# rlvc/FEALESS

Hardware: AMD Instinct MI355X
Metric: frames/sec (640x480 RGB-D x N templates, 20 ICP iters) (higher is better)
Workload: dtype u8

## Files before the change

fealess_amd/csrc/fl_frontend.hip:

```cpp
#include "fl_internal.h"
#include <float.h>

#ifndef FL_CQ_DOT4
#define FL_CQ_DOT4 1
#endif

__device__ __forceinline__ int clampi(int v, int lo, int hi) { return v < lo ? lo : (v > hi ? hi : v); }
__device__ __forceinline__ int reflect101(int p, int len)
{
  if (len == 1) return 0;
  while (p < 0 || p >= len) p = p < 0 ? -p : 2 * len - 2 - p;
  return p;
}

__device__ __forceinline__ float fast_atan2_deg(float y, float x)
{
  const float p1 = 0.9997878412794807f * (float)(180 / 3.14159265358979323846);
  const float p3 = -0.3258083974640975f * (float)(180 / 3.14159265358979323846);
  const float p5 = 0.1555786518463281f * (float)(180 / 3.14159265358979323846);
  const float p7 = -0.04432655554792128f * (float)(180 / 3.14159265358979323846);
  const float ax = fabsf(x), ay = fabsf(y);
  const bool steep = !(ax >= ay);
  const float c = (steep ? ax : ay) / ((steep ? ay : ax) + (float)DBL_EPSILON);
  const float c2 = c * c;
  const float poly = (((p7 * c2 + p5) * c2 + p3) * c2 + p1) * c;
  float a = steep ? 90.f - poly : poly;
  if (x < 0) a = 180.f - a;
  if (y < 0) a = 360.f - a;
  return a;
}

#define CQ_COLS 60
#define CQ_CH 60

__device__ __forceinline__ unsigned wave_from_prev(unsigned v) { return (unsigned)__builtin_amdgcn_update_dpp((int)v, (int)v, 0x138, 0xF, 0xF, false); }
__device__ __forceinline__ unsigned wave_from_next(unsigned v) { return (unsigned)__builtin_amdgcn_update_dpp((int)v, (int)v, 0x130, 0xF, 0xF, false); }
__device__ __forceinline__ unsigned wave_from_prev0(unsigned v) { return (unsigned)__builtin_amdgcn_update_dpp(0, (int)v, 0x138, 0xF, 0xF, true); }
__device__ __forceinline__ unsigned wave_from_next0(unsigned v) { return (unsigned)__builtin_amdgcn_update_dpp(0, (int)v, 0x130, 0xF, 0xF, true); }

__host__ __device__ __forceinline__ void cq_window_addr(uint32_t row_mis, int w, int xc, uint32_t *off, uint32_t *shift, int *first)
{
  const int f = xc - 3 < 0 ? 0 : (xc - 3 > w - 7 ? w - 7 : xc - 3);
  const uint32_t o = row_mis + 3u * (uint32_t)f;
  *off = o & ~3u;
  *shift = o & 3u;
  *first = f;
}

__host__ __device__ __forceinline__ uint32_t cq_alignbyte(uint32_t hi, uint32_t lo, uint32_t s)
{
#if defined(__HIP_DEVICE_COMPILE__)
  return __builtin_amdgcn_alignbyte(hi, lo, s);
#else
  return (uint32_t)((((uint64_t)hi << 32) | lo) >> (8 * (s & 3u)));
#endif
}

__host__ __device__ __forceinline__ void cq_window(const uint8_t *__restrict__ row4, uint32_t row_mis, int w, int xc, bool any_left,
                                                   bool any_right, uint32_t *wd)
{
  uint32_t off, shift;
  int first;
  cq_window_addr(row_mis, w, xc, &off, &shift, &first);
  const int dpx = xc - 3 - first;
  uint32_t d[6];
  const uint8_t *q = (const uint8_t *)__builtin_assume_aligned(row4 + off, 4);
  __builtin_memcpy(d, q, 16);
  __builtin_memcpy(d + 4, q + 16, 8);
#pragma unroll
  for (int k = 0; k < 5; ++k) wd[k] = cq_alignbyte(d[k + 1], d[k], shift);
  wd[5] = cq_alignbyte(d[5], d[5], shift);
#define CQ_TAKE(e0, e1, e2, e3, e4, e5, e6, e7, e8)                                                                                 \
  {                                                                                                                                 \
    const bool b0 = (dw & 1u) != 0u, b1 = (dw & 2u) != 0u;                                                                          \
    const uint32_t t0 = b0 ? e1 : e0, t1 = b0 ? e2 : e1, t2 = b0 ? e3 : e2, t3 = b0 ? e4 : e3, t4 = b0 ? e5 : e4, t5 = b0 ? e6 : e5, \
                   t6 = b0 ? e7 : e6, t7 = b0 ? e8 : e7;                                                                            \
    const uint32_t g0 = b1 ? t2 : t0, g1 = b1 ? t3 : t1, g2 = b1 ? t4 : t2, g3 = b1 ? t5 : t3, g4 = b1 ? t6 : t4, g5 = b1 ? t7 : t5; \
    wd[0] = cq_alignbyte(g1, g0, s);                                                                                                \
    wd[1] = cq_alignbyte(g2, g1, s);                                                                                                \
    wd[2] = cq_alignbyte(g3, g2, s);                                                                                                \
    wd[3] = cq_alignbyte(g4, g3, s);                                                                                                \
    wd[4] = cq_alignbyte(g5, g4, s);                                                                                                \
    wd[5] = cq_alignbyte(g5, g5, s);                                                                                                \
  }
  if (any_left) {
    const uint32_t s = dpx < 0 ? (uint32_t)-dpx : 0u, dw = 3u - s;
    const uint32_t p = wd[0] & 0xFFFFFFu;
    CQ_TAKE((p | (p << 24)), ((p >> 8) | (p << 16)), ((p >> 16) | (p << 8)), wd[0], wd[1], wd[2], wd[3], wd[4], wd[5])
  }
  if (any_right) {
    const uint32_t n = dpx > 0 ? 3u * (uint32_t)dpx : 0u, dw = n >> 2, s = n & 3u;
    const uint32_t p = (wd[4] >> 16) | ((wd[5] & 0xFFu) << 16);
    CQ_TAKE(wd[0], wd[1], wd[2], wd[3], wd[4], ((p >> 16) | (p << 8)), (p | (p << 24)), ((p >> 8) | (p << 16)), 0u)
  }
#undef CQ_TAKE
}

template <bool kNarrow>
__device__ __forceinline__ void cq_hrow(const uint8_t *__restrict__ src, int w, int h, int row, int xc, bool any_left, bool any_right,
                                        int *h3)
{
  const int kk[7] = {8, 28, 56, 72, 56, 28, 8};
  const uint8_t *p = src + (size_t)clampi(row, 0, h - 1) * (size_t)(w * 3);
  int a0 = 0, a1 = 0, a2 = 0;
  if (!kNarrow) {
    const uint32_t mis = (uint32_t)(uintptr_t)p & 3u;
    uint32_t wd[6];
    cq_window(p - mis, mis, w, xc, any_left, any_right, wd);
#if FL_CQ_DOT4
    unsigned acc[3] = {0u, 0u, 0u};
#pragma unroll
    for (int ch = 0; ch < 3; ++ch)
#pragma unroll
      for (int k = 0; k < 6; ++k) {
        unsigned wk = 0;
#pragma unroll
        for (int t = 0; t < 7; ++t)
          if (((3 * t + ch) >> 2) == k) wk |= (unsigned)kk[t] << (8 * ((3 * t + ch) & 3));
        if (wk != 0u) acc[ch] = __builtin_amdgcn_udot4(wd[k], wk, acc[ch], false);
      }
    a0 = (int)acc[0]; a1 = (int)acc[1]; a2 = (int)acc[2];
#else
#pragma unroll
    for (int t = 0; t < 7; ++t) {
      const int b0 = 3 * t, b1 = 3 * t + 1, b2 = 3 * t + 2;
      a0 += kk[t] * (int)((wd[b0 >> 2] >> (8 * (b0 & 3))) & 0xFFu);
      a1 += kk[t] * (int)((wd[b1 >> 2] >> (8 * (b1 & 3))) & 0xFFu);
      a2 += kk[t] * (int)((wd[b2 >> 2] >> (8 * (b2 & 3))) & 0xFFu);
    }
#endif
  } else {
#pragma unroll
    for (int t = 0; t < 7; ++t) {
      const uint8_t *q = p + 3 * clampi(xc + t - 3, 0, w - 1);
      a0 += kk[t] * q[0];
      a1 += kk[t] * q[1];
      a2 += kk[t] * q[2];
    }
  }
  h3[0] = a0;
  h3[1] = a1;
  h3[2] = a2;
}

extern "C" void fl_dev_cq_window_addr(unsigned row_mis, int w, int xc, unsigned *off, unsigned *shift, int *first)
{
  cq_window_addr(row_mis, w, xc, off, shift, first);
}
extern "C" void fl_dev_cq_window_taps(const uint8_t *row4, unsigned row_mis, int w, int xc, int any_left, int any_right, uint8_t *taps21)
{
  uint32_t wd[6];
  cq_window(row4, row_mis, w, xc, any_left != 0, any_right != 0, wd);
  for (int b = 0; b < 21; ++b) taps21[b] = (uint8_t)(wd[b >> 2] >> (8 * (b & 3)));
}

#ifndef FL_CQ_WPE
#define FL_CQ_WPE 6
#endif
template <bool kMag, bool kNarrow>
__global__ __launch_bounds__(256) __attribute__((amdgpu_waves_per_eu(kNarrow ? 6 : FL_CQ_WPE, kNarrow ? 6 : FL_CQ_WPE))) void k_color_quantize(const uint8_t *__restrict__ bgr, size_t in_stride,
                                                        uint8_t *__restrict__ dst, size_t out_stride, int w, int h,
                                                        float threshold_sq, int nstrips, int nchunks, int chunk_rows,
                                                        float *__restrict__ mag_out, const uint32_t *__restrict__ tiles,
                                                        size_t tiles_stride)
{
  const int wave = __builtin_amdgcn_readfirstlane((int)(threadIdx.x >> 6)), lane = threadIdx.x & 63;
  const int item = blockIdx.x * 4 + wave;
  if (item >= nstrips * nchunks) return;
  const int strip = item % nstrips, chunk = item / nstrips;
  int row_lo = 0, row_hi = h - 1;
  if (tiles) {
    const uint32_t *tb = tiles + (size_t)blockIdx.z * tiles_stride;
    const int t = chunk * nstrips + strip;
    if (!((tb[FL_TILE_WORDS + (t >> 5)] >> (t & 31)) & 1u)) return;
    const uint32_t rw = tb[2 * FL_TILE_WORDS + 32 * FL_TILE_WORDS + t];
    row_lo = (int)(rw >> 16);
    row_hi = (int)(rw & 0xFFFFu);
  }
  const uint8_t *src = bgr + (size_t)blockIdx.z * in_stride;
  uint8_t *out = dst + (size_t)blockIdx.z * out_stride;
  const int x = strip * CQ_COLS + lane - 2;
  const int xc = clampi(x, 0, w - 1);
  const int y0 = max(chunk * chunk_rows, row_lo), y1 = min(min(h, chunk * chunk_rows + chunk_rows), row_hi + 1);
  if (y0 >= y1) return;
  const bool any_left = strip == 0, any_right = strip * CQ_COLS + 61 > w - 4;

  int H[7][3];
  {
    const int center = clampi(y0 - 2, 0, h - 1);
#pragma unroll
    for (int i = 0; i < 7; ++i) cq_hrow<kNarrow>(src, w, h, center + i - 3, xc, any_left, any_right, H[i]);
  }
  uint32_t Sl[3] = {0, 0, 0}, Sc[3] = {0, 0, 0}, Sr[3] = {0, 0, 0};
  uint32_t Qp[3] = {0, 0, 0};
  float Mg[3] = {0.f, 0.f, 0.f};
  auto smooth = [&](int p) __attribute__((always_inline)) {
    uint32_t vv[3];
#pragma unroll
    for (int ch = 0; ch < 3; ++ch)
      vv[ch] = __umul24(8u, (unsigned)(H[p % 7][ch] + H[(p + 6) % 7][ch])) + __umul24(28u, (unsigned)(H[(p + 1) % 7][ch] + H[(p + 5) % 7][ch])) +
               __umul24(56u, (unsigned)(H[(p + 2) % 7][ch] + H[(p + 4) % 7][ch])) + __umul24(72u, (unsigned)H[(p + 3) % 7][ch]);
    const uint32_t S = (uint32_t)(((int)vv[0] + (1 << 15)) >> 16) | ((uint32_t)(((int)vv[1] + (1 << 15)) >> 16) << 8) |
                       ((uint32_t)(((int)vv[2] + (1 << 15)) >> 16) << 16);
    const uint32_t L = wave_from_prev0(S), R = wave_from_next0(S);
    Sl[0] = Sl[1]; Sl[1] = Sl[2]; Sl[2] = L;
    Sc[0] = Sc[1]; Sc[1] = Sc[2]; Sc[2] = S;
    Sr[0] = Sr[1]; Sr[1] = Sr[2]; Sr[2] = R;
  };
  auto again = [&]() __attribute__((always_inline)) {
    Sl[0] = Sl[1]; Sl[1] = Sl[2];
    Sc[0] = Sc[1]; Sc[1] = Sc[2];
    Sr[0] = Sr[1]; Sr[1] = Sr[2];
  };
  auto finish = [&](int yv) __attribute__((always_inline)) {
    if (yv < y0) return;
    const int ys = yv - 1;
    int bdx = 0, bdy = 0, bmag = 0;
    {
      int dxs[3], dys[3], mags[3];
#pragma unroll
      for (int ch = 0; ch < 3; ++ch) {
        const int sh = 8 * ch;
#define PX(v) ((int)(((v) >> sh) & 0xFFu))
        const int dx = (PX(Sr[0]) - PX(Sl[0])) + 2 * (PX(Sr[1]) - PX(Sl[1])) + (PX(Sr[2]) - PX(Sl[2]));
        const int dy = (PX(Sl[2]) - PX(Sl[0])) + 2 * (PX(Sc[2]) - PX(Sc[0])) + (PX(Sr[2]) - PX(Sr[0]));
#undef PX
        dxs[ch] = dx;
        dys[ch] = dy;
        mags[ch] = __mul24(dx, dx) + __mul24(dy, dy);
      }
      if (mags[0] >= mags[1] && mags[0] >= mags[2]) { bdx = dxs[0]; bdy = dys[0]; bmag = mags[0]; }
      else if (mags[1] >= mags[0] && mags[1] >= mags[2]) { bdx = dxs[1]; bdy = dys[1]; bmag = mags[1]; }
      else { bdx = dxs[2]; bdy = dys[2]; bmag = mags[2]; }
    }
    const float ang = fast_atan2_deg((float)bdy, (float)bdx);
    int qi = __float2int_rn(ang * (float)(16.0 / 360.0));
    qi = qi < 0 ? 0 : (qi > 255 ? 255 : qi);
    const bool inside = ys > 0 && ys < h - 1 && x > 0 && x < w - 1;
    const uint32_t q = inside ? (uint32_t)(qi & 7) : 0u;
    const uint32_t oh = 1u << (4 * q);
    const uint32_t ohl = wave_from_prev0(oh), ohr = wave_from_next0(oh);
    Qp[0] = Qp[1]; Qp[1] = Qp[2]; Qp[2] = oh + ohl + ohr;
    Mg[0] = Mg[1]; Mg[1] = Mg[2]; Mg[2] = (float)bmag;
    if (yv < y0 + 2) return;
    const int yo = yv - 2;
    if (lane >= 2 && lane < 2 + CQ_COLS && x < w && yo < y1) {
      uint8_t res = 0;
      if (yo >= 1 && yo < h - 1 && x >= 1 && x < w - 1 && Mg[1] > threshold_sq) {
        const unsigned hist = Qp[0] + Qp[1] + Qp[2];
        const unsigned maj = (hist + 0x33333333u) & 0x88888888u;
        if (maj) res = (uint8_t)(1u << ((__ffs((int)maj) - 4) >> 2));
      }
      out[(size_t)yo * w + x] = res;
      if (kMag) mag_out[(size_t)blockIdx.z * out_stride + (size_t)yo * w + x] = Mg[1];
      else if (mag_out) mag_out[(size_t)yo * w + x] = Mg[1];
    }
  };

  const int ylast = y1 + 1, yadv = min(ylast, h - 1);
  int yv = y0 - 2;
  smooth(0);
  for (++yv; yv <= min(ylast, 0); ++yv) {
    again();
    finish(yv);
  }
  for (;;) {
#pragma unroll
    for (int P = 0; P < 7; ++P) {
      if (yv > yadv) goto below;
      cq_hrow<kNarrow>(src, w, h, yv + 3, xc, any_left, any_right, H[P]);
      smooth(P + 1);
      finish(yv);
      ++yv;
    }
  }
below:
  for (; yv <= ylast; ++yv) {
    again();
    finish(yv);
  }
}

int fl_launch_quantized_orientations(fl_context *ctx, const uint8_t *bgr, size_t in_stride, uint8_t *dst,
                                     size_t out_stride, int n_frames, int w, int h, float weak_threshold)
{
  return fl_launch_quantized_orientations_mag(ctx, bgr, in_stride, dst, out_stride, n_frames, w, h, weak_threshold, nullptr);
}

#define FL_CHUNK_FILL 4
template <typename K>
static long waves_per_cu(K kernel, long *cache)
{
  if (*cache == 0) {
    int blocks = 0;
    *cache = hipOccupancyMaxActiveBlocksPerMultiprocessor(&blocks, kernel, 256, 0) == hipSuccess && blocks > 0 ? 4l * blocks : 32;
  }
  return *cache;
}
static int fl_eager_chunk_rows(const fl_context *ctx, long per_cu, int nstrips, int n_frames, int h)
{
  if (ctx->opt.frontend_chunk_rows) return (int)ctx->opt.frontend_chunk_rows;
  const long need = (long)FL_CHUNK_FILL * ctx->cus * per_cu;
  return h > 60 && (long)nstrips * n_frames * ((h + 119) / 120) >= need ? 120 : 60;
}

static_assert(CQ_COLS == FL_TILE && CQ_CH == FL_TILE, "the lazy tile grid is k_color_quantize's work decomposition");
static int launch_color_quantize(fl_context *ctx, const uint8_t *bgr, size_t in_stride, uint8_t *dst, size_t out_stride, int n_frames,
                                 int w, int h, float weak_threshold, float *mag_out, const uint32_t *tiles, size_t tiles_stride)
{
  static long per_cu[4] = {0, 0, 0, 0};
  const int nstrips = (w + CQ_COLS - 1) / CQ_COLS;
  const bool narrow = w < 8;
  auto launch = [&](auto kernel, long *cache) {
    const int rows = tiles ? CQ_CH : fl_eager_chunk_rows(ctx, waves_per_cu(kernel, cache), nstrips, n_frames, h);
    const int nchunks = (h + rows - 1) / rows;
    dim3 grid((nstrips * nchunks + 3) / 4, 1, n_frames);
    hipLaunchKernelGGL(kernel, grid, dim3(256), 0, ctx->stream, bgr, in_stride, dst, out_stride, w, h, weak_threshold * weak_threshold,
                       nstrips, nchunks, rows, mag_out, tiles, tiles_stride);
  };
  if (mag_out) {
    if (narrow) launch(k_color_quantize<true, true>, &per_cu[3]);
    else launch(k_color_quantize<true, false>, &per_cu[1]);
  } else {
    if (narrow) launch(k_color_quantize<false, true>, &per_cu[2]);
    else launch(k_color_quantize<false, false>, &per_cu[0]);
  }
  FL_HIP(ctx, hipGetLastError());
  return FL_OK;
}

int fl_launch_quantized_orientations_mag(fl_context *ctx, const uint8_t *bgr, size_t in_stride, uint8_t *dst,
                                         size_t out_stride, int n_frames, int w, int h, float weak_threshold, float *mag_out)
{
  return launch_color_quantize(ctx, bgr, in_stride, dst, out_stride, n_frames, w, h, weak_threshold, mag_out, nullptr, 0);
}

__device__ __forceinline__ void pyrdown_general_px(const uint8_t *__restrict__ src, int w, int h, int x, int y, uint8_t *o)
{
  const int k[5] = {1, 4, 6, 4, 1};
  int acc0 = 0, acc1 = 0, acc2 = 0;
#pragma unroll
  for (int j = 0; j < 5; ++j) {
    const int yy = reflect101(2 * y + j - 2, h);
    int r0 = 0, r1 = 0, r2 = 0;
#pragma unroll
    for (int i = 0; i < 5; ++i) {
      const int xx = reflect101(2 * x + i - 2, w);
      const uint8_t *p = src + ((size_t)yy * w + xx) * 3;
      r0 += k[i] * p[0];
      r1 += k[i] * p[1];
      r2 += k[i] * p[2];
    }
    acc0 += k[j] * r0;
    acc1 += k[j] * r1;
    acc2 += k[j] * r2;
  }
  o[0] = (uint8_t)((acc0 + 128) >> 8);
  o[1] = (uint8_t)((acc1 + 128) >> 8);
  o[2] = (uint8_t)((acc2 + 128) >> 8);
}

__global__ __launch_bounds__(256) void k_pyrdown_general(const uint8_t *__restrict__ src_, size_t in_stride,
                                                         uint8_t *__restrict__ dst_, size_t out_stride, int w, int h)
{
  const int dw = w / 2, dh = h / 2;
  const int x = blockIdx.x * 32 + (threadIdx.x & 31), y = blockIdx.y * 8 + (threadIdx.x >> 5);
  if (x >= dw || y >= dh) return;
  const uint8_t *src = src_ + (size_t)blockIdx.z * in_stride;
  uint8_t *dst = dst_ + (size_t)blockIdx.z * out_stride;
  pyrdown_general_px(src, w, h, x, y, dst + ((size_t)y * dw + x) * 3);
}

#define PD_ROWS 8
__global__ __launch_bounds__(256) void k_pyrdown_pairs(const uint8_t *__restrict__ src_, size_t in_stride,
                                                       uint8_t *__restrict__ dst_, size_t out_stride, int w, int h)
{
  const int dw = w / 2, dh = h / 2, np = dw / 2;
  const int per = (np + (int)gridDim.x - 1) / (int)gridDim.x, lane = threadIdx.x & 63;
  const int xp = blockIdx.x * per + lane;
  const int y0 = (blockIdx.y * 4 + (threadIdx.x >> 6)) * PD_ROWS;
  if (lane >= per || xp >= np || y0 >= dh) return;
  const uint8_t *src = src_ + (size_t)blockIdx.z * in_stride;
  uint8_t *dst = dst_ + (size_t)blockIdx.z * out_stride;
  const bool first = xp == 0, last = xp == np - 1;
  const bool wave_first = blockIdx.x == 0, wave_last = blockIdx.x == gridDim.x - 1;
  const int off16 = first ? 0 : 12 * xp - 8, off8 = first ? 16 : (last ? 12 * xp + 4 : 12 * xp + 8);
  auto hrow = [&](int r, int (&o)[6]) {
    const int yy = reflect101(r, h);
    uint32_t wd[6];
    const uint8_t *p = src + (size_t)yy * w * 3;
    __builtin_memcpy(wd, p + off16, 16);
    __builtin_memcpy(wd + 4, p + off8, 8);
    if (wave_first) {
      const uint32_t mix = (wd[2] & 0xFFu) | ((wd[0] >> 24) << 8) | (wd[1] << 16);
      const uint32_t n0 = wd[1], n2 = wd[0], n3 = wd[1], n4 = wd[2], n5 = wd[3];
      wd[0] = first ? n0 : wd[0];
      wd[1] = first ? mix : wd[1];
      wd[2] = first ? n2 : wd[2];
      wd[3] = first ? n3 : wd[3];
      wd[4] = first ? n4 : wd[4];
      wd[5] = first ? n5 : wd[5];
    }
    if (wave_last) {
      const uint32_t hi = wd[5];
      wd[4] = last ? hi : wd[4];
      wd[5] = last ? ((wd[3] >> 16) | (hi << 16)) : wd[5];
    }
#define SB(b) ((int)((wd[(b) >> 2] >> (8 * ((b) & 3))) & 0xFFu))
#pragma unroll
    for (int ch = 0; ch < 3; ++ch) {
      o[ch] = SB(2 + ch) + 4 * SB(5 + ch) + 6 * SB(8 + ch) + 4 * SB(11 + ch) + SB(14 + ch);
      o[3 + ch] = SB(8 + ch) + 4 * SB(11 + ch) + 6 * SB(14 + ch) + 4 * SB(17 + ch) + SB(20 + ch);
    }
#undef SB
  };
  int H[5][6];
  hrow(2 * y0 - 2, H[0]);
  hrow(2 * y0 - 1, H[1]);
  hrow(2 * y0, H[2]);
#pragma unroll
  for (int k = 0; k < PD_ROWS; ++k) {
    const int y = y0 + k;
    if (y < dh) {
      hrow(2 * y + 1, H[(2 * k + 3) % 5]);
      hrow(2 * y + 2, H[(2 * k + 4) % 5]);
      uint32_t v[6];
#pragma unroll
      for (int c = 0; c < 6; ++c) {
        const int acc = H[(2 * k) % 5][c] + 4 * H[(2 * k + 1) % 5][c] + 6 * H[(2 * k + 2) % 5][c] + 4 * H[(2 * k + 3) % 5][c] +
                        H[(2 * k + 4) % 5][c];
        v[c] = (uint32_t)((acc + 128) >> 8);
      }
      uint16_t *o = (uint16_t *)(dst + ((size_t)y * dw + 2 * xp) * 3);
      o[0] = (uint16_t)(v[0] | (v[1] << 8));
      o[1] = (uint16_t)(v[2] | (v[3] << 8));
      o[2] = (uint16_t)(v[4] | (v[5] << 8));
    }
  }
}

int fl_launch_pyrdown_bgr(fl_context *ctx, const uint8_t *src, size_t in_stride, uint8_t *dst, size_t out_stride,
                          int n_frames, int w, int h)
{
  const int dw = w / 2, dh = h / 2;
  const bool pairs_ok = dw >= 8 && (w & 1) == 0 && (dw & 1) == 0 && ((3 * dw) & 1) == 0 && (out_stride & 1) == 0 && (((size_t)dst) & 1) == 0;
  if (!pairs_ok) {
    dim3 grid((dw + 31) / 32, (dh + 7) / 8, n_frames);
    hipLaunchKernelGGL(k_pyrdown_general, grid, dim3(256), 0, ctx->stream, src, in_stride, dst, out_stride, w, h);
  } else {
    dim3 grid((dw / 2 + 63) / 64, (dh + 4 * PD_ROWS - 1) / (4 * PD_ROWS), n_frames);
    hipLaunchKernelGGL(k_pyrdown_pairs, grid, dim3(256), 0, ctx->stream, src, in_stride, dst, out_stride, w, h);
  }
  FL_HIP(ctx, hipGetLastError());
  return FL_OK;
}

__constant__ uint8_t c_normal_lut[400];
static bool g_normal_lut_ready[64] = {false};

static int ensure_normal_lut(fl_context *ctx)
{
  if (ctx->device < 64 && g_normal_lut_ready[ctx->device]) return FL_OK;
  uint8_t lut[400];
  for (int y = 0; y < 20; ++y)
    for (int x = 0; x < 20; ++x) {
      double best = -1e300;
      int bk = 0;
      for (int k = 0; k < 8; ++k) {
        double a = k * (3.14159265358979323846 / 4);
        double d = (x - 10) * cos(a) + (y - 10) * sin(a);
        if (d > best + 1e-9) { best = d; bk = k; }
      }
      lut[y * 20 + x] = (uint8_t)(1 << bk);
    }
  FL_HIP(ctx, hipMemcpyToSymbol(HIP_SYMBOL(c_normal_lut), lut, sizeof(lut)));
  if (ctx->device < 64) g_normal_lut_ready[ctx->device] = true;
  return FL_OK;
}

#define DQ_COLS 60

__device__ __forceinline__ unsigned dq_pattern(unsigned cls) { return cls >= 8u ? 0u : 0x11111111u << (4u * cls); }

__device__ __forceinline__ unsigned dq_normal_pattern(const uint16_t *__restrict__ depth, int w, int h, int y, int x,
                                                      int distance_threshold, int difference_threshold, const uint8_t *lut)
{
  const int r = 5;
  if (!(y >= r && y < h - r - 1 && x >= r && x < w - r - 1)) return dq_pattern(0);
  const uint16_t *p = depth + (__umul24((unsigned)y, (unsigned)w) + (unsigned)x);
  const int d = p[0];
  if (!(d < distance_threshold)) return dq_pattern(0);
  const int t = difference_threshold;
  const unsigned span = t > 0 ? (unsigned)(2 * t - 1) : 0u;
  const int e0 = (int)p[-r - r * w] - d, e1 = (int)p[0 - r * w] - d, e2 = (int)p[+r - r * w] - d, e3 = (int)p[-r] - d,
            e4 = (int)p[+r] - d, e5 = (int)p[-r + r * w] - d, e6 = (int)p[0 + r * w] - d, e7 = (int)p[+r + r * w] - d;
  const bool g0 = (unsigned)(e0 + t - 1) < span, g1 = (unsigned)(e1 + t - 1) < span,
             g2 = (unsigned)(e2 + t - 1) < span, g3 = (unsigned)(e3 + t - 1) < span,
             g4 = (unsigned)(e4 + t - 1) < span, g5 = (unsigned)(e5 + t - 1) < span,
             g6 = (unsigned)(e6 + t - 1) < span, g7 = (unsigned)(e7 + t - 1) < span;
  const int f0 = g0, f1 = g1, f2 = g2, f3 = g3, f4 = g4, f5 = g5, f6 = g6, f7 = g7;
  const int m0 = g0 ? e0 : 0, m1 = g1 ? e1 : 0, m2 = g2 ? e2 : 0, m3 = g3 ? e3 : 0, m4 = g4 ? e4 : 0, m5 = g5 ? e5 : 0,
            m6 = g6 ? e6 : 0, m7 = g7 ? e7 : 0;
  const int corners = f0 + f2 + f5 + f7;
  const int A0 = __mul24(25, corners + f3 + f4), A3 = __mul24(25, corners + f1 + f6), A1 = __mul24(25, (f0 + f7) - (f2 + f5));
  const int det = __mul24(A0, A3) - __mul24(A1, A1);
  float nx, ny, nz;
  if (t <= 400) {
    const int b0 = __mul24(5, (m2 + m4 + m7) - (m0 + m3 + m5)), b1 = __mul24(5, (m5 + m6 + m7) - (m0 + m1 + m2));
    const int ddx = __mul24(A3, b0) - __mul24(A1, b1), ddy = __mul24(A0, b1) - __mul24(A1, b0);
    nx = (float)__mul24(617, ddx);
    ny = (float)__mul24(617, ddy);
    nz = (float)(-__mul24(det, d));
  } else {
    const int b0 = 5 * ((m2 + m4 + m7) - (m0 + m3 + m5)), b1 = 5 * ((m5 + m6 + m7) - (m0 + m1 + m2));
    const long long ddx = (long long)A3 * b0 - (long long)A1 * b1, ddy = -(long long)A1 * b0 + (long long)A0 * b1;
    nx = (float)(617LL * ddx);
    ny = (float)(617LL * ddy);
    nz = (float)(-(long long)det * d);
  }
  const float s = sqrtf(nx * nx + ny * ny + nz * nz);
  if (!(s > 0)) return dq_pattern(0);
  const float inv = 1.0f / s;
  nx *= inv;
  ny *= inv;
  nz *= inv;
  const int v1 = (int)(nx * 10 + 10);
  const int v2 = (int)(ny * 10 + 10);
  const int v3 = (int)(nz * 20 + 20);
  if (!(v1 >= 0 && v1 <= 19 && v2 >= 0 && v2 <= 19 && v3 >= 0 && v3 <= 19)) return dq_pattern(0);
  const unsigned v = lut[v2 * 20 + v1];
  return dq_pattern(v ? (unsigned)(32 - __clz(v)) : 0u);
}

__global__ __launch_bounds__(256) void k_depth_quantize(const uint16_t *__restrict__ depth_, size_t in_stride,
                                                        uint8_t *__restrict__ dst_, size_t out_stride, int w, int h,
                                                        int distance_threshold, int difference_threshold, int nstrips,
                                                        int nchunks, int chunk_rows, uint8_t *__restrict__ dst1_,
                                                        size_t out1_stride)
{
  __shared__ uint8_t s_lut[400];
  for (int k = threadIdx.x; k < 400; k += 256) s_lut[k] = c_normal_lut[k];
  __syncthreads();
  const int wave = threadIdx.x >> 6, lane = threadIdx.x & 63;
  const int item = blockIdx.x * 4 + wave;
  if (item >= nstrips * nchunks) return;
  const int strip = item % nstrips, chunk = item / nstrips;
  const uint16_t *depth = depth_ + (size_t)blockIdx.z * in_stride;
  uint8_t *dst = dst_ + (size_t)blockIdx.z * out_stride;
  uint8_t *dst1 = dst1_ ? dst1_ + (size_t)blockIdx.z * out1_stride : nullptr;
  const int x = strip * DQ_COLS + lane - 2;
  const int xc = clampi(x, 0, w - 1);
  const int y0 = chunk * chunk_rows, y1 = min(h, y0 + chunk_rows);
  unsigned p0 = 0, p1 = 0, p2 = 0, p3 = 0, p4 = 0;
  int center = -1;
  unsigned pat = 0;
  for (int yv = y0 - 2; yv <= y1 + 1; ++yv) {
    const int c = clampi(yv, 0, h - 1);
    if (c != center) {
      pat = dq_normal_pattern(depth, w, h, c, xc, distance_threshold, difference_threshold, s_lut);
      center = c;
    }
    p4 = p3; p3 = p2; p2 = p1; p1 = p0; p0 = pat;
    if (yv < y0 + 2) continue;
    const unsigned col = p0 + p1 + p2 + p3 + p4;
    const unsigned a1 = wave_from_next(col), b1 = wave_from_prev(col), a2 = wave_from_next(a1), b2 = wave_from_prev(b1);
    const unsigned s3 = col + a1 + b1, s2 = a2 + b2;
    const unsigned te = (s3 & 0x0F0F0F0Fu) + (s2 & 0x0F0F0F0Fu) + 0x73737373u;
    const unsigned to = ((s3 >> 4) & 0x0F0F0F0Fu) + ((s2 >> 4) & 0x0F0F0F0Fu) + 0x73737373u;
    const int idx = 8 - __popc((te & 0x80808080u) | ((to & 0x80808080u) >> 1));
    const int yo = yv - 2;
    if (lane >= 2 && lane < 2 + DQ_COLS && x < w) {
      const uint8_t v = idx ? (uint8_t)(1u << (idx - 1)) : 0;
      dst[__umul24((unsigned)yo, (unsigned)w) + (unsigned)x] = v;
      if (dst1 && !((yo | x) & 1)) dst1[__umul24((unsigned)yo >> 1, (unsigned)w >> 1) + ((unsigned)x >> 1)] = v;
    }
  }
}

int fl_launch_quantized_normals(fl_context *ctx, const uint16_t *depth, size_t in_stride, uint8_t *dst,
                                size_t out_stride, uint8_t *dst1, size_t out1_stride, int n_frames, int w, int h,
                                int distance_threshold, int difference_threshold)
{
  static long per_cu = 0;
  int rc = ensure_normal_lut(ctx);
  if (rc) return rc;
  if (dst1 && ((w | h) & 1)) return fl_set_error(ctx, FL_ERR_INVALID, "fused half-size normals need even sizes, got %dx%d", w, h);
  const int nstrips = (w + DQ_COLS - 1) / DQ_COLS;
  const int rows = fl_eager_chunk_rows(ctx, waves_per_cu(k_depth_quantize, &per_cu), nstrips, n_frames, h);
  const int nchunks = (h + rows - 1) / rows;
  dim3 grid((nstrips * nchunks + 3) / 4, 1, n_frames);
  hipLaunchKernelGGL(k_depth_quantize, grid, dim3(256), 0, ctx->stream, depth, in_stride / sizeof(uint16_t), dst, out_stride,
                     w, h, distance_threshold, difference_threshold, nstrips, nchunks, rows, dst1, out1_stride);
  FL_HIP(ctx, hipGetLastError());
  return FL_OK;
}

__global__ __launch_bounds__(256) void k_resize_nn_half4(const uint8_t *__restrict__ src_, size_t in_stride,
                                                         uint8_t *__restrict__ dst_, size_t out_stride, int w, int h)
{
  const int dw = w / 2, dh = h / 2;
  const int x4 = blockIdx.x * 64 + (threadIdx.x & 63), y = blockIdx.y * 4 + (threadIdx.x >> 6);
  if (4 * x4 >= dw || y >= dh) return;
  const uint8_t *src = src_ + (size_t)blockIdx.z * in_stride;
  uint8_t *dst = dst_ + (size_t)blockIdx.z * out_stride;
  uint2 v;
  __builtin_memcpy(&v, __builtin_assume_aligned(src + (size_t)(2 * y) * w + 8 * x4, 8), 8);
  const uint32_t o = (v.x & 0xFFu) | ((v.x >> 8) & 0xFF00u) | ((v.y & 0xFFu) << 16) | ((v.y << 8) & 0xFF000000u);
  *(uint32_t *)(dst + (size_t)y * dw + 4 * x4) = o;
}

__global__ __launch_bounds__(256) void k_resize_nn_half(const uint8_t *__restrict__ src_, size_t in_stride,
                                                        uint8_t *__restrict__ dst_, size_t out_stride, int w, int h)
{
  const int dw = w / 2, dh = h / 2;
  const int x = blockIdx.x * 64 + (threadIdx.x & 63), y = blockIdx.y * 4 + (threadIdx.x >> 6);
  if (x >= dw || y >= dh) return;
  const uint8_t *src = src_ + (size_t)blockIdx.z * in_stride;
  uint8_t *dst = dst_ + (size_t)blockIdx.z * out_stride;
  int sx = (int)floor(x * (1.0 / ((double)dw / w))), sy = (int)floor(y * (1.0 / ((double)dh / h)));
  sx = min(sx, w - 1);
  sy = min(sy, h - 1);
  dst[(size_t)y * dw + x] = src[(size_t)sy * w + sx];
}

static bool resize_nn_half_fast(const uint8_t *src, size_t in_stride, const uint8_t *dst, size_t out_stride, int w, int h)
{
  return (w % 8) == 0 && (h % 2) == 0 && ((in_stride | out_stride) & 7) == 0 && ((((size_t)src) | ((size_t)dst)) & 7) == 0;
}

int fl_launch_resize_nn_half(fl_context *ctx, const uint8_t *src, size_t in_stride, uint8_t *dst, size_t out_stride,
                             int n_frames, int w, int h)
{
  if (resize_nn_half_fast(src, in_stride, dst, out_stride, w, h)) {
    dim3 grid((w / 8 + 63) / 64, (h / 2 + 3) / 4, n_frames);
    hipLaunchKernelGGL(k_resize_nn_half4, grid, dim3(256), 0, ctx->stream, src, in_stride, dst, out_stride, w, h);
  } else {
    dim3 grid((w / 2 + 63) / 64, (h / 2 + 3) / 4, n_frames);
    hipLaunchKernelGGL(k_resize_nn_half, grid, dim3(256), 0, ctx->stream, src, in_stride, dst, out_stride, w, h);
  }
  FL_HIP(ctx, hipGetLastError());
  return FL_OK;
}

struct FlFrontImages {
  int L, M;
  int w[FL_MAX_LEVELS], h[FL_MAX_LEVELS];
  uint8_t *bgr[FL_MAX_LEVELS], *qcolor[FL_MAX_LEVELS], *qdepth[FL_MAX_LEVELS];
  size_t stride;
};
static int launch_front_images(fl_context *ctx, const FlFrontImages &im, int n_frames, const uint8_t *bgr, size_t bgr_stride,
                               const uint16_t *depth, size_t depth_stride, int first_color_level)
{
  int rc;
  bool fused1 = false;
  for (int l = 0; l < im.L; ++l) {
    if (l > 0) {
      rc = fl_launch_pyrdown_bgr(ctx, l == 1 ? bgr : im.bgr[l - 1], l == 1 ? bgr_stride : im.stride, im.bgr[l], im.stride, n_frames,
                                 im.w[l - 1], im.h[l - 1]);
      if (rc) return rc;
      if (im.M > 1 && !(l == 1 && fused1)) {
        rc = fl_launch_resize_nn_half(ctx, im.qdepth[l - 1], im.stride, im.qdepth[l], im.stride, n_frames, im.w[l - 1], im.h[l - 1]);
        if (rc) return rc;
      }
    } else if (im.M > 1) {
      fused1 = im.L > 1 && resize_nn_half_fast(im.qdepth[0], im.stride, im.qdepth[1], im.stride, im.w[0], im.h[0]);
      rc = fl_launch_quantized_normals(ctx, depth, depth_stride, im.qdepth[0], im.stride, fused1 ? im.qdepth[1] : nullptr, im.stride,
                                       n_frames, im.w[0], im.h[0], 2000, 50);
      if (rc) return rc;
    }
    if (l < first_color_level) continue;
    rc = fl_launch_quantized_orientations(ctx, l == 0 ? bgr : im.bgr[l], l == 0 ? bgr_stride : im.stride, im.qcolor[l], im.stride,
                                          n_frames, im.w[l], im.h[l], 10.0f);
    if (rc) return rc;
  }
  return FL_OK;
}

int fl_launch_frontend(fl_detector *det, int n_frames, const uint8_t *bgr, size_t bgr_stride, const uint16_t *depth,
                       size_t depth_stride, bool allow_lazy)
{
  fl_context *ctx = det->ctx;
  det->lazy = allow_lazy && det->lazy_capable && !det->eager_env;
  det->lazy_bgr = bgr;
  det->lazy_bgr_stride = bgr_stride;
  FlFrontImages im;
  im.L = det->L;
  im.M = det->M;
  im.stride = det->ws_stride;
  for (int l = 0; l < det->L; ++l) {
    const FlLevelGeom &g = det->geom[l];
    im.w[l] = g.w;
    im.h[l] = g.h;
    im.bgr[l] = det->d_ws + g.bgr_off;
    im.qcolor[l] = det->d_ws + g.quant_off[0];
    im.qdepth[l] = det->d_ws + g.quant_off[1];
  }
  int rc = launch_front_images(ctx, im, n_frames, bgr, bgr_stride, depth, depth_stride, det->lazy ? det->L - 1 : 0);
  if (rc) return rc;
  if (det->have_times) FL_HIP(ctx, hipEventRecord(det->ev[1], ctx->stream));
  return FL_OK;
}

extern "C" int fl_dev_front_images(fl_context *ctx, const uint8_t *bgr, const uint16_t *depth, int n_frames, int w, int h, int levels,
                                   uint8_t *out, size_t out_bytes)
{
  if (!ctx || !bgr || !depth || !out || n_frames < 1 || levels < 1 || levels > FL_MAX_LEVELS || w < 3 || h < 3 || (w >> (levels - 1)) < 3 ||
      (h >> (levels - 1)) < 3)
    return FL_ERR_INVALID;
  FL_HIP(ctx, hipSetDevice(ctx->device));
  FlFrontImages im;
  im.L = levels;
  im.M = 2;
  size_t off = 0;
  for (int l = 0; l < levels; ++l) {
    im.w[l] = w >> l;
    im.h[l] = h >> l;
    const size_t px = (size_t)im.w[l] * im.h[l];
    im.qcolor[l] = (uint8_t *)off;
    im.qdepth[l] = (uint8_t *)(off + fl_align(px, 256));
    im.bgr[l] = (uint8_t *)(off + 2 * fl_align(px, 256));
    off += 2 * fl_align(px, 256) + (l ? fl_align(3 * px, 256) : 0);
  }
  const size_t packed = off, fb = (size_t)w * h * 3, fd = (size_t)w * h * 2, in_b = fl_align(fb * n_frames, 256);
  size_t need = 0;
  for (int l = 0; l < levels; ++l) need += (size_t)im.w[l] * im.h[l] * (l ? 5 : 2);
  if (out_bytes < need * n_frames) return fl_set_error(ctx, FL_ERR_INVALID, "fl_dev_front_images: out holds %zu bytes, %zu needed", out_bytes, need * n_frames);
  void *s = nullptr;
  int rc = fl_scratch(ctx, in_b + fl_align(fd * n_frames, 256) + packed * n_frames, &s);
  if (rc) return rc;
  uint8_t *d_bgr = (uint8_t *)s, *d_depth = d_bgr + in_b, *d_im = d_depth + fl_align(fd * n_frames, 256);
  im.stride = packed;
  for (int l = 0; l < levels; ++l) {
    im.qcolor[l] = d_im + (size_t)im.qcolor[l];
    im.qdepth[l] = d_im + (size_t)im.qdepth[l];
    im.bgr[l] = d_im + (size_t)im.bgr[l];
  }
  FL_HIP(ctx, hipMemcpyAsync(d_bgr, bgr, fb * n_frames, hipMemcpyHostToDevice, ctx->stream));
  FL_HIP(ctx, hipMemcpyAsync(d_depth, depth, fd * n_frames, hipMemcpyHostToDevice, ctx->stream));
  FL_HIP(ctx, hipMemsetAsync(d_im, 0xFF, packed * n_frames, ctx->stream));
  if ((rc = launch_front_images(ctx, im, n_frames, d_bgr, fb, (const uint16_t *)d_depth, fd, 0))) return rc;
  for (int f = 0; f < n_frames; ++f)
    for (int l = 0; l < levels; ++l) {
      const size_t px = (size_t)im.w[l] * im.h[l];
      FL_HIP(ctx, hipMemcpyAsync(out, im.qcolor[l] + f * packed, px, hipMemcpyDeviceToHost, ctx->stream));
      FL_HIP(ctx, hipMemcpyAsync(out + px, im.qdepth[l] + f * packed, px, hipMemcpyDeviceToHost, ctx->stream));
      if (l) FL_HIP(ctx, hipMemcpyAsync(out + 2 * px, im.bgr[l] + f * packed, 3 * px, hipMemcpyDeviceToHost, ctx->stream));
      out += (l ? 5 : 2) * px;
    }
  FL_HIP(ctx, hipStreamSynchronize(ctx->stream));
  return FL_OK;
}

int fl_launch_lazy_level(fl_detector *det, int n_frames, int level)
{
  fl_context *ctx = det->ctx;
  const FlLevelGeom &g = det->geom[level];
  const uint32_t *tiles = (const uint32_t *)(det->d_ws + det->off_tiles) + (size_t)level * FL_TILE_BLOCK_WORDS;
  const size_t tstride = det->ws_stride / sizeof(uint32_t);
  if (det->poison_env) {
    FL_HIP(ctx, hipMemset2DAsync(det->d_ws + g.quant_off[0], det->ws_stride, 0xFF, (size_t)g.w * g.h, n_frames, ctx->stream));
    for (int m = 0; m < det->M; ++m)
      FL_HIP(ctx, hipMemset2DAsync(det->d_ws + g.spread_off[m], det->ws_stride, 0xFF, (size_t)g.w * g.h, n_frames, ctx->stream));
  }
  int rc = launch_color_quantize(ctx, level == 0 ? det->lazy_bgr : det->d_ws + g.bgr_off, level == 0 ? det->lazy_bgr_stride : det->ws_stride,
                                 det->d_ws + g.quant_off[0], det->ws_stride, n_frames, g.w, g.h, 10.0f, nullptr,
                                 tiles, tstride);
  if (rc) return rc;
  for (int m = 0; m < det->M; ++m) {
    rc = fl_launch_spread_tiles(ctx, det->d_ws + g.quant_off[m], det->ws_stride, det->d_ws + g.spread_off[m], det->ws_stride, n_frames,
                                g.w, g.h, g.T, tiles, tstride);
    if (rc) return rc;
  }
  return FL_OK;
}

template <typename F>
static int run_stage(fl_context *ctx, const void *in, size_t in_bytes, void *out, size_t out_bytes, size_t tmp_bytes,
                     int mem, F body)
{
  FL_HIP(ctx, hipSetDevice(ctx->device));
  const uint8_t *din = (const uint8_t *)in;
  uint8_t *dout = (uint8_t *)out, *dtmp = nullptr;
  void *s = nullptr;
  size_t need = fl_align(tmp_bytes, 256) + (mem == FL_MEM_HOST ? fl_align(in_bytes, 256) + fl_align(out_bytes, 256) : 0);
  if (need) {
    int rc = fl_scratch(ctx, need, &s);
    if (rc) return rc;
  }
  dtmp = (uint8_t *)s;
  if (mem == FL_MEM_HOST) {
    uint8_t *b = (uint8_t *)s + fl_align(tmp_bytes, 256);
    FL_HIP(ctx, hipMemcpyAsync(b, in, in_bytes, hipMemcpyHostToDevice, ctx->stream));
    din = b;
    dout = b + fl_align(in_bytes, 256);
  }
  int rc = body(din, dout, dtmp);
  if (rc) return rc;
  if (mem == FL_MEM_HOST) {
    FL_HIP(ctx, hipMemcpyAsync(out, dout, out_bytes, hipMemcpyDeviceToHost, ctx->stream));
    FL_HIP(ctx, hipStreamSynchronize(ctx->stream));
  }
  return FL_OK;
}

extern "C" int fl_quantized_orientations(fl_context *ctx, const uint8_t *bgr, int w, int h, float weak_threshold,
                                         uint8_t *dst, int mem)
{
  if (!ctx || !bgr || !dst || w < 3 || h < 3) return FL_ERR_INVALID;
  return run_stage(ctx, bgr, (size_t)w * h * 3, dst, (size_t)w * h, 0, mem,
                   [&](const uint8_t *i, uint8_t *o, uint8_t *) {
                     return fl_launch_quantized_orientations(ctx, i, 0, o, 0, 1, w, h, weak_threshold);
                   });
}

extern "C" int fl_quantized_normals(fl_context *ctx, const uint16_t *depth, int w, int h, int distance_threshold,
                                    int difference_threshold, uint8_t *dst, int mem)
{
  if (!ctx || !depth || !dst || w <= 0 || h <= 0) return FL_ERR_INVALID;
  return run_stage(ctx, depth, (size_t)w * h * 2, dst, (size_t)w * h, (size_t)w * h, mem,
                   [&](const uint8_t *i, uint8_t *o, uint8_t *) {
                     return fl_launch_quantized_normals(ctx, (const uint16_t *)i, 0, o, 0, nullptr, 0, 1, w, h,
                                                        distance_threshold, difference_threshold);
                   });
}

extern "C" int fl_pyrdown_bgr(fl_context *ctx, const uint8_t *src, int w, int h, uint8_t *dst, int mem)
{
  if (!ctx || !src || !dst || w < 2 || h < 2) return FL_ERR_INVALID;
  return run_stage(ctx, src, (size_t)w * h * 3, dst, (size_t)(w / 2) * (h / 2) * 3, 0, mem,
                   [&](const uint8_t *i, uint8_t *o, uint8_t *) { return fl_launch_pyrdown_bgr(ctx, i, 0, o, 0, 1, w, h); });
}

struct FlResizeTap { int ofs; float w0, w1; };
__device__ __forceinline__ FlResizeTap fl_resize_tap(int d, int ssize, double scale)
{
  float f = (float)((d + 0.5) * scale - 0.5);
  int s = (int)floorf(f);
  f -= (float)s;
  if (s < 0) { f = 0.f; s = 0; }
  if (s >= ssize - 1) { f = 0.f; s = ssize - 1; }
  return {s, 1.f - f, f};
}
__device__ __forceinline__ int fl_sat_short(float v)
{
  const int r = (int)rintf(v);
  return r < -32768 ? -32768 : r > 32767 ? 32767 : r;
}

template <typename T, int CN>
__global__ __launch_bounds__(256) void k_resize_linear(const T *__restrict__ src, int sw, int sh, T *__restrict__ dst, int dw,
                                                       int dh, double scale_x, double scale_y, int area2)
{
  const int x = blockIdx.x * 64 + (threadIdx.x & 63), y = blockIdx.y * 4 + (threadIdx.x >> 6);
  if (x >= dw || y >= dh) return;
  if (area2) {
    const T *s0 = src + ((size_t)(2 * y) * sw + 2 * x) * CN, *s1 = s0 + (size_t)sw * CN;
#pragma unroll
    for (int c = 0; c < CN; ++c) dst[((size_t)y * dw + x) * CN + c] = (T)(((int)s0[c] + s0[CN + c] + s1[c] + s1[CN + c] + 2) >> 2);
    return;
  }
  const FlResizeTap ty = fl_resize_tap(y, sh, scale_y), tx = fl_resize_tap(x, sw, scale_x);
  const int y0 = ty.ofs, y1 = min(ty.ofs + 1, sh - 1), x0 = tx.ofs, x1 = min(tx.ofs + 1, sw - 1);
  const T *r0 = src + (size_t)y0 * sw * CN, *r1 = src + (size_t)y1 * sw * CN;
  if (sizeof(T) == 1) {
    const int a0 = fl_sat_short(tx.w0 * 2048.f), a1 = fl_sat_short(tx.w1 * 2048.f);
    const int b0 = fl_sat_short(ty.w0 * 2048.f), b1 = fl_sat_short(ty.w1 * 2048.f);
#pragma unroll
    for (int c = 0; c < CN; ++c) {
      const int S0 = (int)r0[x0 * CN + c] * a0 + (int)r0[x1 * CN + c] * a1;
      const int S1 = (int)r1[x0 * CN + c] * a0 + (int)r1[x1 * CN + c] * a1;
      dst[((size_t)y * dw + x) * CN + c] = (T)((((b0 * (S0 >> 4)) >> 16) + ((b1 * (S1 >> 4)) >> 16) + 2) >> 2);
    }
  } else {
#pragma unroll
    for (int c = 0; c < CN; ++c) {
      float S0 = (float)r0[x0 * CN + c] * tx.w0;
      S0 = S0 + (float)r0[x1 * CN + c] * tx.w1;
      float S1 = (float)r1[x0 * CN + c] * tx.w0;
      S1 = S1 + (float)r1[x1 * CN + c] * tx.w1;
      float v = S0 * ty.w0;
      v = v + S1 * ty.w1;
      const int r = (int)rintf(v);
      dst[((size_t)y * dw + x) * CN + c] = (T)(r < 0 ? 0 : r > 65535 ? 65535 : r);
    }
  }
}

template <typename T, int CN>
static int fl_resize_linear(fl_context *ctx, const T *src, int sw, int sh, T *dst, int dw, int dh, int mem)
{
  if (!ctx || !src || !dst || sw < 1 || sh < 1 || dw < 1 || dh < 1) return FL_ERR_INVALID;
  const double scale_x = (double)sw / dw, scale_y = (double)sh / dh;
  const int area2 = fabs(scale_x - 2.0) < 2.220446049250313e-16 && fabs(scale_y - 2.0) < 2.220446049250313e-16;
  return run_stage(ctx, src, (size_t)sw * sh * CN * sizeof(T), dst, (size_t)dw * dh * CN * sizeof(T), 0, mem,
                   [&](const uint8_t *i, uint8_t *o, uint8_t *) {
                     hipLaunchKernelGGL((k_resize_linear<T, CN>), dim3((dw + 63) / 64, (dh + 3) / 4), dim3(256), 0, ctx->stream,
                                        (const T *)i, sw, sh, (T *)o, dw, dh, scale_x, scale_y, area2);
                     FL_HIP(ctx, hipGetLastError());
                     return (int)FL_OK;
                   });
}

int fl_launch_resize_linear_bgr8(fl_context *ctx, const uint8_t *src, int sw, int sh, uint8_t *dst, int dw, int dh)
{
  return fl_resize_linear<uint8_t, 3>(ctx, src, sw, sh, dst, dw, dh, FL_MEM_DEVICE);
}
int fl_launch_resize_linear_u16(fl_context *ctx, const uint16_t *src, int sw, int sh, uint16_t *dst, int dw, int dh)
{
  return fl_resize_linear<uint16_t, 1>(ctx, src, sw, sh, dst, dw, dh, FL_MEM_DEVICE);
}

extern "C" int fl_resize_linear_bgr8(fl_context *ctx, const uint8_t *src, int sw, int sh, uint8_t *dst, int dw, int dh, int mem)
{
  return fl_resize_linear<uint8_t, 3>(ctx, src, sw, sh, dst, dw, dh, mem);
}

extern "C" int fl_resize_linear_u16(fl_context *ctx, const uint16_t *src, int sw, int sh, uint16_t *dst, int dw, int dh, int mem)
{
  return fl_resize_linear<uint16_t, 1>(ctx, src, sw, sh, dst, dw, dh, mem);
}
```

Before: 80870.

## Cache depth taps in register ring buffer for normal quantization sweep

Rewrites the per-column vertical sweep in the depth quantize kernel to keep an 11-row register ring of left/center/right depth taps, loading only one new row per step instead of eight neighbour taps per pixel. The loop is unrolled by the ring length with compile-time phase indices, and output pointers are advanced incrementally rather than recomputed. It also makes the wave index scalar. This cuts redundant global loads and address arithmetic, at the cost of more registers and more complex boundary handling at the top and bottom rows.

```diff
diff --git a/fealess_amd/csrc/fl_frontend.hip b/fealess_amd/csrc/fl_frontend.hip
--- a/fealess_amd/csrc/fl_frontend.hip
+++ b/fealess_amd/csrc/fl_frontend.hip
@@ -1,5 +1,6 @@
 #include "fl_internal.h"
 #include <float.h>
+#include <type_traits>
 
 #ifndef FL_CQ_DOT4
 #define FL_CQ_DOT4 1
@@ -482,18 +483,14 @@
 
 __device__ __forceinline__ unsigned dq_pattern(unsigned cls) { return cls >= 8u ? 0u : 0x11111111u << (4u * cls); }
 
-__device__ __forceinline__ unsigned dq_normal_pattern(const uint16_t *__restrict__ depth, int w, int h, int y, int x,
-                                                      int distance_threshold, int difference_threshold, const uint8_t *lut)
-{
-  const int r = 5;
-  if (!(y >= r && y < h - r - 1 && x >= r && x < w - r - 1)) return dq_pattern(0);
-  const uint16_t *p = depth + (__umul24((unsigned)y, (unsigned)w) + (unsigned)x);
-  const int d = p[0];
+__device__ __forceinline__ unsigned dq_normal_pattern(bool interior, int d, int n0, int n1, int n2, int n3, int n4, int n5, int n6,
+                                                      int n7, int distance_threshold, int difference_threshold, const uint8_t *lut)
+{
+  if (!interior) return dq_pattern(0);
   if (!(d < distance_threshold)) return dq_pattern(0);
   const int t = difference_threshold;
   const unsigned span = t > 0 ? (unsigned)(2 * t - 1) : 0u;
-  const int e0 = (int)p[-r - r * w] - d, e1 = (int)p[0 - r * w] - d, e2 = (int)p[+r - r * w] - d, e3 = (int)p[-r] - d,
-            e4 = (int)p[+r] - d, e5 = (int)p[-r + r * w] - d, e6 = (int)p[0 + r * w] - d, e7 = (int)p[+r + r * w] - d;
+  const int e0 = n0 - d, e1 = n1 - d, e2 = n2 - d, e3 = n3 - d, e4 = n4 - d, e5 = n5 - d, e6 = n6 - d, e7 = n7 - d;
   const bool g0 = (unsigned)(e0 + t - 1) < span, g1 = (unsigned)(e1 + t - 1) < span,
              g2 = (unsigned)(e2 + t - 1) < span, g3 = (unsigned)(e3 + t - 1) < span,
              g4 = (unsigned)(e4 + t - 1) < span, g5 = (unsigned)(e5 + t - 1) < span,
@@ -532,6 +529,8 @@
   return dq_pattern(v ? (unsigned)(32 - __clz(v)) : 0u);
 }
 
+#define DQ_RING 11
+
 __global__ __launch_bounds__(256) void k_depth_quantize(const uint16_t *__restrict__ depth_, size_t in_stride,
                                                         uint8_t *__restrict__ dst_, size_t out_stride, int w, int h,
                                                         int distance_threshold, int difference_threshold, int nstrips,
@@ -541,7 +540,7 @@
   __shared__ uint8_t s_lut[400];
   for (int k = threadIdx.x; k < 400; k += 256) s_lut[k] = c_normal_lut[k];
   __syncthreads();
-  const int wave = threadIdx.x >> 6, lane = threadIdx.x & 63;
+  const int wave = __builtin_amdgcn_readfirstlane((int)(threadIdx.x >> 6)), lane = threadIdx.x & 63;
   const int item = blockIdx.x * 4 + wave;
   if (item >= nstrips * nchunks) return;
   const int strip = item % nstrips, chunk = item / nstrips;
@@ -551,17 +550,29 @@
   const int x = strip * DQ_COLS + lane - 2;
   const int xc = clampi(x, 0, w - 1);
   const int y0 = chunk * chunk_rows, y1 = min(h, y0 + chunk_rows);
+  unsigned ol = 2u * (unsigned)max(xc - 5, 0), oc = 2u * (unsigned)xc, orr = 2u * (unsigned)min(xc + 5, w - 1);
+  unsigned ox = (unsigned)x, ox1 = (unsigned)x >> 1;
+  auto lane_off = [](unsigned &off) __attribute__((always_inline)) { asm volatile("" : "+v"(off)); return off; };
+  auto tap = [&](const char *rowp, unsigned &off) __attribute__((always_inline)) { return (int)*(const uint16_t *)(rowp + lane_off(off)); };
+  const bool xin = xc >= 5 && xc < w - 6;
+  const bool writes = lane >= 2 && lane < 2 + DQ_COLS && x < w;
+  const int cs = max(y0 - 2, 0), ce = min(y1 + 1, h - 1);
+  const size_t row_bytes = 2 * (size_t)w;
+  int RL[DQ_RING], RC[DQ_RING], RR[DQ_RING];
+#pragma unroll
+  for (int i = 0; i < DQ_RING - 1; ++i) {
+    const char *rowp = (const char *)depth + (size_t)clampi(cs + i - 5, 0, h - 1) * row_bytes;
+    RL[i] = tap(rowp, ol);
+    RC[i] = tap(rowp, oc);
+    RR[i] = tap(rowp, orr);
+  }
+  const char *ldp = (const char *)depth + (size_t)min(cs + 5, h - 1) * row_bytes;
+  uint8_t *orow = dst + (size_t)y0 * (size_t)w;
+  uint8_t *orow1 = dst1 ? dst1 + (size_t)(y0 >> 1) * (size_t)(w >> 1) : nullptr;
   unsigned p0 = 0, p1 = 0, p2 = 0, p3 = 0, p4 = 0;
-  int center = -1;
-  unsigned pat = 0;
-  for (int yv = y0 - 2; yv <= y1 + 1; ++yv) {
-    const int c = clampi(yv, 0, h - 1);
-    if (c != center) {
-      pat = dq_normal_pattern(depth, w, h, c, xc, distance_threshold, difference_threshold, s_lut);
-      center = c;
-    }
-    p4 = p3; p3 = p2; p2 = p1; p1 = p0; p0 = pat;
-    if (yv < y0 + 2) continue;
+  auto push = [&](unsigned pat) __attribute__((always_inline)) { p4 = p3; p3 = p2; p2 = p1; p1 = p0; p0 = pat; };
+  auto finish = [&](int yv) __attribute__((always_inline)) {
+    if (yv < y0 + 2) return;
     const unsigned col = p0 + p1 + p2 + p3 + p4;
     const unsigned a1 = wave_from_next(col), b1 = wave_from_prev(col), a2 = wave_from_next(a1), b2 = wave_from_prev(b1);
     const unsigned s3 = col + a1 + b1, s2 = a2 + b2;
@@ -569,11 +580,37 @@
     const unsigned to = ((s3 >> 4) & 0x0F0F0F0Fu) + ((s2 >> 4) & 0x0F0F0F0Fu) + 0x73737373u;
     const int idx = 8 - __popc((te & 0x80808080u) | ((to & 0x80808080u) >> 1));
     const int yo = yv - 2;
-    if (lane >= 2 && lane < 2 + DQ_COLS && x < w) {
+    if (writes) {
       const uint8_t v = idx ? (uint8_t)(1u << (idx - 1)) : 0;
-      dst[__umul24((unsigned)yo, (unsigned)w) + (unsigned)x] = v;
-      if (dst1 && !((yo | x) & 1)) dst1[__umul24((unsigned)yo >> 1, (unsigned)w >> 1) + ((unsigned)x >> 1)] = v;
-    }
+      orow[lane_off(ox)] = v;
+      if (orow1 && !((yo | x) & 1)) orow1[lane_off(ox1)] = v;
+    }
+    orow += w;
+    if (orow1 && (yo & 1)) orow1 += w >> 1;
+  };
+  int yv = y0 - 2;
+  for (; yv < 0; ++yv) push(dq_pattern(0));
+  auto step = [&](auto phase) __attribute__((always_inline)) {
+    constexpr int P = decltype(phase)::value, A = P % DQ_RING, C = (P + 5) % DQ_RING, B = (P + 10) % DQ_RING;
+    RL[B] = tap(ldp, ol);
+    RC[B] = tap(ldp, oc);
+    RR[B] = tap(ldp, orr);
+    if (yv + 5 < h - 1) ldp += row_bytes;
+    push(dq_normal_pattern(xin && yv >= 5 && yv < h - 6, RC[C], RL[A], RC[A], RR[A], RL[C], RR[C], RL[B], RC[B], RR[B],
+                           distance_threshold, difference_threshold, s_lut));
+    finish(yv);
+    ++yv;
+  };
+#define DQ_STEP(P)                                                                                                                  \
+  if (yv > ce) break;                                                                                                               \
+  step(std::integral_constant<int, P>());
+  for (;;) {
+    DQ_STEP(0) DQ_STEP(1) DQ_STEP(2) DQ_STEP(3) DQ_STEP(4) DQ_STEP(5) DQ_STEP(6) DQ_STEP(7) DQ_STEP(8) DQ_STEP(9) DQ_STEP(10)
+  }
+#undef DQ_STEP
+  for (; yv <= y1 + 1; ++yv) {
+    push(dq_pattern(0));
+    finish(yv);
   }
 }
 
```

Result: faster. 81930 (median of 6 runs) (+1.3%).
